# joaospinto/sip_optimal_control

Hardware: AMD Instinct MI355X
Metric: Riccati sweeps/sec (backward+forward) (higher is better)
Workload: dtype f64

## Files before the change

sip_optimal_control_amd/csrc/kkt_chain_kernels.hpp:

```cpp
#pragma once
#include <hip/hip_runtime.h>

#include <cstdint>

#include "kkt_kernels.hpp"

namespace sipamd {
namespace kkt {

struct ChainKkt {
  int n, m, T, cn, gn, cT, gT, ce, ge;
  int node_len, edge_len;
  long model_len;
  int x_dim, y_dim, z_dim;
  int mats_stage, vecs_stage;
  long mats_len, vecs_len;
  int lds_item, lds_tail, lds_rows;
  int split;
  int sym;
};

typedef double d2_t __attribute__((ext_vector_type(2)));

template <int FN, int FM>
// ... 104 lines not shown
    for (int u = 0; u < U; ++u)
      if (tid + u * TPB < n0)
        da[tid + u * TPB] = va[u];
#pragma unroll
    for (int u = 0; u < U; ++u)
      if (tid + u * TPB < n1)
        db[tid + u * TPB] = vb[u];
  } else {
    stage_copy2(d0, s0, l0, tid);
    stage_copy2(d1, s1, l1, tid);
  }
}

typedef double d4_t __attribute__((ext_vector_type(4)));

struct CondenseItem {
  long p;
  int i;
  bool last;
  int c, g, ce, ge, nrows, node_len, edge_len;
  int y_dyn, y_nc, y_ec, z_n, z_e;
  const double *item, *r1, *yinv, *zinv, *b, *b_y, *b_z;
  double *mats, *vecs;
};

template <bool WITH_RHS>
__device__ __forceinline__ CondenseItem condense_item(const ChainKkt &ck, const long p, const int i,
                                                      const double *model_all, const double *r1_all,
                                                      const double *inv_all, double *mats_all, const double *b_all,
                                                      double *vecs_all) {
  CondenseItem it;
  const int n = ck.n, m = ck.m, T = ck.T;
  it.p = p, it.i = i, it.last = i == T;
  it.c = it.last ? ck.cT : ck.cn, it.g = it.last ? ck.gT : ck.gn;
  it.ce = it.last ? 0 : ck.ce, it.ge = it.last ? 0 : ck.ge;
  it.nrows = it.c + it.g + it.ce + it.ge;
  it.node_len = n * n + (it.c + it.g) * n, it.edge_len = it.last ? 0 : ck.edge_len;
  const long kkt = (long)ck.x_dim + ck.y_dim + ck.z_dim;
  it.item = model_all + p * ck.model_len + (long)i * (ck.node_len + ck.edge_len);
  it.r1 = r1_all != nullptr ? r1_all + p * ck.x_dim + i * (n + m) : nullptr;
  it.yinv = inv_all + p * ((long)ck.y_dim + ck.z_dim), it.zinv = it.yinv + ck.y_dim;
  it.y_dyn = i * (n + ck.cn), it.y_nc = it.y_dyn + n, it.y_ec = T * (n + ck.cn) + n + ck.cT + i * ck.ce;
  it.z_n = i * ck.gn, it.z_e = T * ck.gn + ck.gT + i * ck.ge;
  it.b = WITH_RHS ? b_all + p * kkt : nullptr;
  it.b_y = WITH_RHS ? it.b + ck.x_dim : nullptr, it.b_z = WITH_RHS ? it.b_y + ck.y_dim : nullptr;
  it.mats = mats_all + p * ck.mats_len + (long)i * ck.mats_stage;
  it.vecs = WITH_RHS ? vecs_all + p * ck.vecs_len + (long)i * ck.vecs_stage : nullptr;
  return it;
}

__device__ __forceinline__ double condense_rhs_row(const CondenseItem &it, const int k, const double *by,
                                                   const double *bz) {
  if (k < it.c)
    return by[it.y_nc + k];
  if (k < it.c + it.g)
    return bz[it.z_n + (k - it.c)];
  if (k < it.c + it.g + it.ce)
    return by[it.y_ec + (k - it.c - it.g)];
  return bz[it.z_e + (k - it.c - it.g - it.ce)];
}
__device__ __forceinline__ double condense_weight_row(const CondenseItem &it, const int k) {
  if (k < it.c)
    return it.yinv[it.y_nc + k];
  if (k < it.c + it.g)
    return it.zinv[it.z_n + (k - it.c)];
  if (k < it.c + it.g + it.ce)
    return it.yinv[it.y_ec + (k - it.c - it.g)];
  return it.zinv[it.z_e + (k - it.c - it.g - it.ce)];
}

struct CondensePre {
  double w, b, q, dy, d, r1;
};

template <bool WITH_RHS, bool MATS>
__device__ __forceinline__ void condense_prefetch(const ChainKkt &ck, const CondenseItem &it, const int tid,
                                                  CondensePre &pre) {
  const int n = ck.n, m = ck.m;
  pre.w = pre.b = pre.q = pre.dy = pre.d = pre.r1 = 0.0;
  if (tid < it.nrows) {
    pre.w = condense_weight_row(it, tid);
    if (WITH_RHS)
      pre.b = condense_rhs_row(it, tid, it.b_y, it.b_z);
  }
  if (MATS) {
    if (tid < n)
      pre.d = it.yinv[it.y_dyn + tid];
    if (tid < (it.last ? n : n + m))
      pre.r1 = it.r1[tid];
  }
  if (WITH_RHS) {
    if (tid < n) {
      pre.q = it.b[it.i * (n + m) + tid];
      pre.dy = it.b_y[it.y_dyn + tid];
    } else if (!it.last && tid >= 32 && tid - 32 < m) {
      pre.q = it.b[it.i * (n + m) + n + (tid - 32)];
    }
  }
}

template <bool WITH_RHS, bool MATS>
__device__ __forceinline__ void condense_commit(const ChainKkt &ck, const CondenseItem &it, const int tid,
                                                const CondensePre &pre, double *wl, double *wr, double *r1s) {
  if (tid < it.nrows) {
    wl[tid] = pre.w;
    if (WITH_RHS)
      wr[tid] = pre.w * pre.b;
  }
  for (int k = tid + TPB; k < it.nrows; k += TPB) {
    const double wk = condense_weight_row(it, k);
    wl[k] = wk;
    if (WITH_RHS)
      wr[k] = wk * condense_rhs_row(it, k, it.b_y, it.b_z);
  }
  if (MATS && tid < (it.last ? ck.n : ck.n + ck.m))
    r1s[tid] = pre.r1;
}

template <bool WITH_RHS, bool MATS>
__device__ __forceinline__ void condense_compute(const ChainKkt &ck, const CondenseItem &it, const int tid,
                                                 const CondensePre &pre, const double *buf, const double *wl,
                                                 double *wr, const double *r1s, const int ncols_rhs,
                                                 const long b_col_stride, const long vecs_col_stride,
                                                 double *obuf = nullptr) {
  const int n = ck.n, m = ck.m, nn = n * n, nm = n * m;
  const bool last = it.last;
  const int c = it.c, g = it.g, ce = it.ce, ge = it.ge;
  const double *Jc = MATS ? buf + nn : buf, *Jg = Jc + c * n;
  const double *eb = buf + it.node_len;
  const int o_m = nn, o_r = o_m + nm, o_a = o_r + m * m, o_b = o_a + nn, o_j = o_b + nm;
  const double *Jxc = MATS ? eb + o_j : buf + (c + g) * n, *Juc = Jxc + ce * n, *Jxg = Juc + ce * m, *Jug = Jxg + ge * n;
  double *mats = MATS ? obuf : it.mats;

  if (MATS)
  {
    const int li = tid & 15, lg = tid >> 4;
    const int ncols = last ? n : n + m;
    const int nt = (ncols + 15) >> 4;
    const bool sym = ck.sym != 0;
// ... 147 lines not shown
        if (!last) {
          acc = dot_seq<true>(acc, Jxc + ce * tid, wr_e, ce);
          acc = dot_seq<true>(acc, Jxg + ge * tid, wr_e + ce, ge);
        }
        vc[tid] = acc;
        vc[n + tid] = -(col == 0 ? pre.dy : bc_y[it.y_dyn + tid]);
      } else if (!last && tid >= 32 && tid - 32 < m) {
        const int d = tid - 32;
        double acc = -(col == 0 ? pre.q : bc[i * (n + m) + n + d]);
        acc = dot_seq<true>(acc, Juc + ce * d, wr_e, ce);
        acc = dot_seq<true>(acc, Jug + ge * d, wr_e + ce, ge);
        vc[2 * n + d] = acc;
      }
    }
  }
}

#ifndef SIP_KKT_RHS_WAVES
#define SIP_KKT_RHS_WAVES 8
#endif
template <bool WITH_RHS, bool MATS = true, int FN = 0, int FM = 0>
__global__ void __launch_bounds__(TPB) __attribute__((amdgpu_waves_per_eu(FN > 0 && !MATS ? SIP_KKT_RHS_WAVES : 1, 8)))
condense_chain_kernel(const ChainKkt ck_in, const double *__restrict__ model_all, const double *__restrict__ r1_all,
                      const double *__restrict__ inv_all, double *__restrict__ mats_all,
                      const double *__restrict__ b_all, double *__restrict__ vecs_all, long batch,
                      const int32_t *__restrict__ status = nullptr, const int ncols = 1,
                      const long b_col_stride = 0, const long vecs_col_stride = 0) {
  static_assert(MATS || WITH_RHS, "nothing to do");
  const ChainKkt ck = family_dims<FN, FM>(ck_in);
  extern __shared__ double sm[];
  double *buf = sm, *wl = buf + (MATS ? ck.lds_item : ck.lds_tail), *wr = wl + ck.lds_rows,
         *r1s = wr + (long)(MATS || ncols < 1 ? 1 : ncols) * ck.lds_rows;
  double *obuf = r1s + ((ck.n + ck.m + 1) & ~1);
  const long p = blockIdx.x / (ck.T + 1);
  const int i = blockIdx.x - (unsigned)(p * (ck.T + 1));
  if (p >= batch || (!MATS && status != nullptr && status[p] != 0))
    return;
  const int tid = threadIdx.x;
  const CondenseItem it = condense_item<WITH_RHS>(ck, p, i, model_all, r1_all, inv_all, mats_all, b_all, vecs_all);
  CondensePre pre;
  condense_prefetch<WITH_RHS, MATS>(ck, it, tid, pre);
  if (MATS) {
    stage_copy2(buf, it.item, it.node_len + it.edge_len, tid);
  } else {
    const int n = ck.n, m = ck.m, nn = n * n;
    const int o_tail = it.node_len + 2 * nn + 2 * n * m + m * m;
    if (it.last)
      stage_copy2(buf, it.item + nn, (it.c + it.g) * n, tid);
    else
      stage_copy_pair(buf, it.item + nn, (it.c + it.g) * n, buf + (it.c + it.g) * n, it.item + o_tail,
                      (it.ce + it.ge) * (n + m), tid);
  }
  condense_commit<WITH_RHS, MATS>(ck, it, tid, pre, wl, wr, r1s);
  __syncthreads();
  condense_compute<WITH_RHS, MATS>(ck, it, tid, pre, buf, wl, wr, r1s, ncols, b_col_stride, vecs_col_stride, obuf);
}

#ifdef SIP_KKT_STAMPS
__device__ unsigned long long g_kkt_seg[16];
#define KKT_SEG(k)                                                                                   \
  do {                                                                                               \
    const unsigned long long now_ = __builtin_amdgcn_s_memtime();                                    \
    seg[k] += now_ - seg_last;                                                                       \
    seg_last = now_;                                                                                 \
  } while (0)
#else
#define KKT_SEG(k)                                                                                   \
  do {                                                                                               \
  } while (0)
#endif
constexpr int PIPE_U = 8;
#ifndef SIP_KKT_PIPE_WAVES
#define SIP_KKT_PIPE_WAVES 1
#endif
template <bool WITH_RHS, int FN = 0, int FM = 0>
__global__ void __launch_bounds__(TPB) __attribute__((amdgpu_waves_per_eu(FN > 0 ? SIP_KKT_PIPE_WAVES : 1, 8)))
condense_chain_pipe_kernel(const ChainKkt ck_in, const double *__restrict__ model_all,
                           const double *__restrict__ r1_all, const double *__restrict__ inv_all,
                           double *__restrict__ mats_all, const double *__restrict__ b_all,
                           double *__restrict__ vecs_all, const long batch, const int per_block) {
  const ChainKkt ck = family_dims<FN, FM>(ck_in);
  extern __shared__ double sm[];
  double *buf = sm, *wl = buf + ck.lds_item, *wr = wl + ck.lds_rows, *r1s = wr + ck.lds_rows;
  double *obuf = r1s + ((ck.n + ck.m + 1) & ~1);
  const int tid = threadIdx.x;
  const long total = batch * (ck.T + 1);
  const long first = (long)blockIdx.x * per_block;
  const long end = first + per_block < total ? first + per_block : total;
  if (first >= end)
    return;
  long walk_p = first / (ck.T + 1);
  int walk_i = (int)(first - walk_p * (ck.T + 1));
  auto item_here = [&]() {
    return condense_item<WITH_RHS>(ck, walk_p, walk_i, model_all, r1_all, inv_all, mats_all, b_all, vecs_all);
  };
  auto step_walk = [&]() {
    if (++walk_i > ck.T)
      walk_i = 0, ++walk_p;
  };
  const int ab_at = ck.node_len + ck.n * ck.n + ck.n * ck.m + ck.m * ck.m;
  const int ab_first = ck.split ? (ab_at + 1) >> 1 : 0;
  const int ab_end = ck.split ? (ab_at + ck.n * ck.n + ck.n * ck.m) >> 1 : 0;
  auto image_load = [&](const CondenseItem &it, d2_t (&v)[PIPE_U]) {
    typedef d2_t d2u_t __attribute__((aligned(8)));
    const d2u_t *s2 = (const d2u_t *)it.item;
    const int len2 = (it.node_len + it.edge_len + 1) >> 1;
#pragma unroll
    for (int u = 0; u < PIPE_U; ++u) {
      int q = min(tid + u * TPB, len2 - 1);
      if (!it.last && q >= ab_first && q < ab_end)
        q = ab_first - 1;
      v[u] = s2[q];
    }
  };
#ifdef SIP_KKT_STAMPS
  unsigned long long seg[8] = {0, 0, 0, 0, 0, 0, 0, 0}, seg_last = __builtin_amdgcn_s_memtime();
#endif
// ... 23 lines not shown
      condense_prefetch<WITH_RHS, true>(ck, cur, tid, pre);
      image_load(cur, img);
    }
    KKT_SEG(3);
    condense_compute<WITH_RHS, true>(ck, nowit, tid, now, buf, wl, wr, r1s, 1, 0, 0, obuf);
    KKT_SEG(4);
    __syncthreads();
    KKT_SEG(5);
  }
#ifdef SIP_KKT_STAMPS
  if (tid == 0)
    for (int k = 0; k < 8; ++k)
      atomicAdd(&g_kkt_seg[k], seg[k]);
#endif
}

#ifndef SIP_KKT_RECOVER_WAVES
#define SIP_KKT_RECOVER_WAVES 8
#endif
template <bool COLS = false, int FN = 0, int FM = 0>
__global__ void __launch_bounds__(TPB) __attribute__((amdgpu_waves_per_eu(FN > 0 && !COLS ? SIP_KKT_RECOVER_WAVES : 1, 8)))
recover_chain_kernel(const ChainKkt ck_in, const double *__restrict__ model_all, const double *__restrict__ b_all,
                     const double *__restrict__ inv_all, const double *__restrict__ lqr_sol_all,
                     double *__restrict__ sol_all, const int32_t *__restrict__ status, long batch,
                     const int ncols = 1, const long b_col_stride = 0, const long lqr_col_stride = 0,
                     const long sol_col_stride = 0) {
  const ChainKkt ck = family_dims<FN, FM>(ck_in);
  extern __shared__ double sm[];
  const int n = ck.n, m = ck.m, T = ck.T;
  const long p = blockIdx.x / (T + 1);
  const int i = blockIdx.x - (unsigned)(p * (T + 1));
  if (p >= batch || status[p] != 0)
    return;
  const int tid = threadIdx.x;
  const bool last = i == T;
  const int c = last ? ck.cT : ck.cn, g = last ? ck.gT : ck.gn;
  const int ce = last ? 0 : ck.ce, ge = last ? 0 : ck.ge;
  const int nn = n * n, nm = n * m;
  const long kkt = (long)ck.x_dim + ck.y_dim + ck.z_dim;
  const double *item = model_all + p * ck.model_len + (long)i * (ck.node_len + ck.edge_len);
  const double *yinv = inv_all + p * ((long)ck.y_dim + ck.z_dim), *zinv = yinv + ck.y_dim;
  const int y_dyn = i * (n + ck.cn), y_nc = y_dyn + n, y_ec = T * (n + ck.cn) + n + ck.cT + i * ck.ce;
  const int z_n = i * ck.gn, z_e = T * ck.gn + ck.gT + i * ck.ge;
  double *jn = sm, *je = jn + (c + g) * n, *xs = sm + ck.lds_tail, *us = xs + n;
  double pre_x = 0.0, pre_y = 0.0, pre_bn = 0.0, pre_wn = 0.0, pre_be = 0.0, pre_we = 0.0;
  {
    const double *b_y = b_all + p * kkt + ck.x_dim, *b_z = b_y + ck.y_dim;
    const double *ls = lqr_sol_all + p * ck.vecs_len + (long)i * ck.vecs_stage;
    if (tid < n) {
      pre_x = ls[tid];
      pre_y = ls[n + tid];
    } else if (!last && tid >= 32 && tid - 32 < m) {
      pre_x = ls[2 * n + (tid - 32)];
    }
    if (tid < c)
      pre_bn = b_y[y_nc + tid], pre_wn = yinv[y_nc + tid];
    else if (tid < c + g)
// ... 407 lines not shown
```

sip_optimal_control_amd/csrc/kkt_kernels.hpp:

```cpp
#pragma once
#include <hip/hip_runtime.h>

#include <cstdint>

namespace sipamd {
namespace kkt {

constexpr int TPB = 64;

enum Block {
  N_Q = 0, N_JC, N_JG, E_Q, E_M, E_R, E_A, E_B, E_JXC, E_JUC, E_JXG, E_JUG, NUM_BLOCKS
};

struct Meta {
  int E, N, root;
  int x_dim, y_dim, z_dim;
  int theta_dim;
  long model_len, in0_len, in1_len, out_len;
  const int *sd, *cd, *ncd, *ngd, *ecd, *egd, *parent, *child, *in_edge, *child_offsets, *child_edges;
  const int *x_state, *x_control, *y_dyn, *y_node_c, *y_edge_c, *z_node, *z_edge;
  const int *y_is_dyn;
  const long *mo[NUM_BLOCKS];
  int lds_q, lds_item, lds_tail, lds_rows;
  const long *oQ, *od, *oq, *oc, *ox, *oy, *oA, *oB, *oM, *oR, *orr, *ou;
// ... 7 lines not shown
  const long idx = (long)blockIdx.x * blockDim.x + threadIdx.x;
  if (idx >= batch * per)
    return;
  const long p = idx / per;
  const int k = (int)(idx - p * per);
  double reg, out;
  if (k < mt.y_dim) {
    reg = r2[p * mt.y_dim + k];
    out = mt.y_is_dyn[k] ? reg : 1.0 / reg;
  } else {
    const long at = p * mt.z_dim + (k - mt.y_dim);
    reg = w[at] + r3[at];
    out = 1.0 / reg;
  }
  inv[idx] = out;
  if (reg <= 0.0)
    atomicOr(&regstat[p], 1);
}

__global__ void __launch_bounds__(256)
merge_status_kernel(const int *__restrict__ regstat, int32_t *__restrict__ status, long batch, int code) {
  const long p = (long)blockIdx.x * blockDim.x + threadIdx.x;
  if (p < batch && regstat[p] != 0)
    status[p] = code;
}

__device__ __forceinline__ double rank_update(double acc, const double *Ja, int ca, const double *Jb, int cb,
                                              int rows, const double *wgt) {
  for (int k = 0; k < rows; ++k)
    acc += (wgt[k] * Jb[k + (long)rows * cb]) * Ja[k + (long)rows * ca];
  return acc;
}

__global__ void __launch_bounds__(TPB)
condense_kernel(const Meta mt, const double *__restrict__ model_all, const double *__restrict__ r1_all,
                const double *__restrict__ inv_all, double *__restrict__ in0_all, long batch) {
  const int items = mt.N + mt.E;
  const long p = blockIdx.x / items;
  const int item = blockIdx.x - (unsigned)(p * items);
  if (p >= batch)
    return;
  const double *model = model_all + p * mt.model_len;
  const double *r1 = r1_all + p * mt.x_dim;
  const double *yinv = inv_all + p * ((long)mt.y_dim + mt.z_dim), *zinv = yinv + mt.y_dim;
  double *in0 = in0_all + p * mt.in0_len;
  const int tid = threadIdx.x;
// ... 612 lines not shown
```

sip_optimal_control_amd/csrc/sip_kkt_amd.hip:

```cpp
#include "../../include/sip_kkt_amd.h"

#include <hip/hip_runtime.h>

#include <algorithm>
#include <cstdio>
#include <cstdlib>
#include <cstring>
#include <new>
#include <string>
#include <type_traits>
#include <vector>

#include "generic_plan.hpp"
#include "stream_fill.hpp"
#include "kkt_chain_kernels.hpp"
#include "kkt_kernels.hpp"
#include "kkt_theta_kernels.hpp"
#include "kkt_theta_chain_kernels.hpp"

struct sip_kkt_plan {
  int64_t batch = 0;
  int device = 0;
  int E = 0, N = 0, root = 0;
  int input_status = SIP_KKT_INVALID_INPUT;
// ... 128 lines not shown
    break;
  switch (family) {
    SIP_KKT_FAMILY_CASE(4, 1) SIP_KKT_FAMILY_CASE(4, 2) SIP_KKT_FAMILY_CASE(4, 3) SIP_KKT_FAMILY_CASE(4, 4)
    SIP_KKT_FAMILY_CASE(6, 1) SIP_KKT_FAMILY_CASE(6, 2) SIP_KKT_FAMILY_CASE(6, 3) SIP_KKT_FAMILY_CASE(6, 4)
    SIP_KKT_FAMILY_CASE(8, 1) SIP_KKT_FAMILY_CASE(8, 2) SIP_KKT_FAMILY_CASE(8, 3) SIP_KKT_FAMILY_CASE(8, 4)
    SIP_KKT_FAMILY_CASE(12, 1) SIP_KKT_FAMILY_CASE(12, 2) SIP_KKT_FAMILY_CASE(12, 3) SIP_KKT_FAMILY_CASE(12, 4)
  default:
    at(std::integral_constant<int, 0>{}, std::integral_constant<int, 0>{});
  }
#undef SIP_KKT_FAMILY_CASE
}

hipError_t launch_condense(const sip_kkt_plan *p, const Regions &r, const double *model, const double *w,
                           const double *r1, const double *r2, const double *r3, const double *b,
                           hipStream_t s, const bool split = false, const bool sym = false) {
  sipamd::kkt::ChainKkt ck = p->ck;
  if (split) {
    const int n = ck.n, m = ck.m;
    const int qlen = sym ? n * (n + 1) / 2 : n * n, rlen = sym ? m * (m + 1) / 2 : m * m;
    ck.split = 1, ck.sym = sym ? 1 : 0;
    ck.mats_stage = (qlen + n) + (n * m + rlen);
    ck.mats_len = (long)(ck.T + 1) * (qlen + n) + (long)ck.T * (n * m + rlen);
  }
  hipError_t e = sipamd::zero_async(r.reg, (size_t)p->batch * sizeof(int), s);
  if (e != hipSuccess)
    return e;
  const long per = (long)p->y_dim + p->z_dim;
  if (per > 0)
    hipLaunchKernelGGL(sipamd::kkt::weights_kernel, dim3((unsigned)((p->batch * per + 255) / 256)), dim3(256), 0, s,
                       p->meta, w, r2, r3, r.inv, r.reg, (long)p->batch);
  const bool pipe = p->chain_kernels && p->chain_pipe > 0 && ((uintptr_t)model & 7) == 0;
  const bool odd_tail = pipe && ((ck.n * ck.n + (ck.cT + ck.gT) * ck.n) & 1);
  const long pipe_batch = odd_tail ? (long)p->batch - 1 : (long)p->batch;
  const unsigned pipe_grid = pipe ? (unsigned)((pipe_batch * p->N + p->chain_pipe - 1) / p->chain_pipe) : 0u;
  const size_t lds_chain = p->chain_kernels ? sizeof(double) * ((size_t)ck.lds_item + 2 * (size_t)ck.lds_rows +
                                                                 (size_t)even(ck.n + ck.m) + (size_t)ck.mats_stage)
                                            : 0;
  auto one_stage = [&](const long q0, const long nb) {
    const long kkt_len = (long)p->x_dim + p->y_dim + p->z_dim;
    const double *mq = model + q0 * ck.model_len, *r1q = r1 + q0 * p->x_dim, *invq = r.inv + q0 * ((long)p->y_dim + p->z_dim);
    double *in0q = r.in0 + q0 * ck.mats_len;
    if (b != nullptr) {
      const double *bq = b + q0 * kkt_len;
      double *in1q = r.in1 + q0 * ck.vecs_len;
      family_dispatch(p->family, [&](auto fn, auto fm) {
        hipLaunchKernelGGL((sipamd::kkt::condense_chain_kernel<true, true, decltype(fn)::value, decltype(fm)::value>),
                           dim3((unsigned)(nb * p->N)), dim3(sipamd::kkt::TPB), lds_chain, s, ck, mq, r1q, invq, in0q, bq,
                           in1q, nb);
      });
    } else {
      family_dispatch(p->family, [&](auto fn, auto fm) {
        hipLaunchKernelGGL((sipamd::kkt::condense_chain_kernel<false, true, decltype(fn)::value, decltype(fm)::value>),
                           dim3((unsigned)(nb * p->N)), dim3(sipamd::kkt::TPB), lds_chain, s, ck, mq, r1q, invq, in0q,
                           (const double *)nullptr, (double *)nullptr, nb);
      });
    }
  };
  if (pipe) {
    if (pipe_batch > 0 && b != nullptr)
      family_dispatch(p->family, [&](auto fn, auto fm) {
        hipLaunchKernelGGL((sipamd::kkt::condense_chain_pipe_kernel<true, decltype(fn)::value, decltype(fm)::value>),
                           dim3(pipe_grid), dim3(sipamd::kkt::TPB), lds_chain, s, ck, model, r1, r.inv, r.in0, b,
                           r.in1, pipe_batch, p->chain_pipe);
      });
    else if (pipe_batch > 0)
      family_dispatch(p->family, [&](auto fn, auto fm) {
        hipLaunchKernelGGL((sipamd::kkt::condense_chain_pipe_kernel<false, decltype(fn)::value, decltype(fm)::value>),
                           dim3(pipe_grid), dim3(sipamd::kkt::TPB), lds_chain, s, ck, model, r1, r.inv, r.in0,
                           (const double *)nullptr, (double *)nullptr, pipe_batch, p->chain_pipe);
      });
    if (odd_tail)
      one_stage((long)p->batch - 1, 1);
  } else if (p->chain_kernels) {
    one_stage(0, (long)p->batch);
  }
  else if (p->staged && b != nullptr)
    hipLaunchKernelGGL(sipamd::kkt::condense_staged_kernel<true>, dim3(node_grid(p)), dim3(sipamd::kkt::TPB),
                       p->lds_condense, s, p->meta, model, r1, r.inv, r.in0, b, r.in1, (long)p->batch);
  else if (p->staged)
    hipLaunchKernelGGL(sipamd::kkt::condense_staged_kernel<false>, dim3(node_grid(p)), dim3(sipamd::kkt::TPB),
                       p->lds_condense, s, p->meta, model, r1, r.inv, r.in0, (const double *)nullptr,
                       (double *)nullptr, (long)p->batch);
  else
    hipLaunchKernelGGL(sipamd::kkt::condense_kernel, dim3(item_grid(p)), dim3(sipamd::kkt::TPB), 0, s, p->meta,
                       model, r1, r.inv, r.in0, (long)p->batch);
  return hipGetLastError();
}

hipError_t launch_merge(const sip_kkt_plan *p, const Regions &r, int32_t *status, hipStream_t s) {
  hipLaunchKernelGGL(sipamd::kkt::merge_status_kernel, dim3((unsigned)((p->batch + 255) / 256)), dim3(256), 0, s,
                     r.reg, status, (long)p->batch, (int)SIP_KKT_NONPOSITIVE_REGULARIZATION);
  return hipGetLastError();
}

hipError_t launch_rhs_meta(const sip_kkt_plan *p, const Meta &mt, const Regions &r, const double *model,
                           const double *b, const int32_t *status, hipStream_t s) {
  if (p->staged)
    hipLaunchKernelGGL(sipamd::kkt::rhs_staged_kernel, dim3(node_grid(p)), dim3(sipamd::kkt::TPB), p->lds_rhs, s,
                       mt, model, b, r.inv, r.in1, status, (long)p->batch);
  else
    hipLaunchKernelGGL(sipamd::kkt::rhs_kernel, dim3(item_grid(p)), dim3(sipamd::kkt::TPB), 0, s, mt, model, b,
                       r.inv, r.in1, status, (long)p->batch);
  return hipGetLastError();
}

hipError_t launch_rhs(const sip_kkt_plan *p, const Regions &r, const double *model, const double *b,
                      const int32_t *status, hipStream_t s) {
  if (p->chain_kernels)
    family_dispatch(p->family, [&](auto fn, auto fm) {
      hipLaunchKernelGGL((sipamd::kkt::condense_chain_kernel<true, false, decltype(fn)::value, decltype(fm)::value>),
                         dim3(node_grid(p)), dim3(sipamd::kkt::TPB),
                         sizeof(double) * ((size_t)p->ck.lds_tail + 2 * (size_t)p->ck.lds_rows), s, p->ck, model,
                         (const double *)nullptr, r.inv, r.in0, b, r.in1, (long)p->batch, status);
    });
  else if (p->staged)
    hipLaunchKernelGGL(sipamd::kkt::rhs_staged_kernel, dim3(node_grid(p)), dim3(sipamd::kkt::TPB), p->lds_rhs, s,
                       p->meta, model, b, r.inv, r.in1, status, (long)p->batch);
  else
    hipLaunchKernelGGL(sipamd::kkt::rhs_kernel, dim3(item_grid(p)), dim3(sipamd::kkt::TPB), 0, s, p->meta, model,
                       b, r.inv, r.in1, status, (long)p->batch);
  return hipGetLastError();
}

hipError_t launch_recover(const sip_kkt_plan *p, const Regions &r, const double *model, const double *b,
                          double *sol, const int32_t *status, hipStream_t s) {
  if (p->chain_kernels)
    family_dispatch(p->family, [&](auto fn, auto fm) {
      hipLaunchKernelGGL((sipamd::kkt::recover_chain_kernel<false, decltype(fn)::value, decltype(fm)::value>),
                         dim3(node_grid(p)), dim3(sipamd::kkt::TPB), p->lds_chain_recover, s, p->ck, model, b, r.inv, r.out,
                         sol, status, (long)p->batch);
    });
  else if (p->staged)
    hipLaunchKernelGGL(sipamd::kkt::recover_staged_kernel, dim3(node_grid(p)), dim3(sipamd::kkt::TPB),
                       p->lds_recover, s, p->meta, model, b, r.inv, r.out, sol, status, (long)p->batch);
  else
    hipLaunchKernelGGL(sipamd::kkt::recover_kernel, dim3(item_grid(p)), dim3(sipamd::kkt::TPB), 0, s, p->meta,
                       model, b, r.inv, r.out, sol, status, (long)p->batch);
  return hipGetLastError();
}

sipamd::kkt::ApplyIO kkt_vector_io(const sip_kkt_plan *p, int theta_dim, const double *d_x, double *d_y) {
  const long xt = (long)p->x_dim + theta_dim, full = xt + p->y_dim + p->z_dim;
  sipamd::kkt::ApplyIO io;
  io.x_x = d_x, io.x_y = d_x + xt, io.x_z = d_x + xt + p->y_dim;
  io.y_x = d_y, io.y_y = d_y + xt, io.y_z = d_y + xt + p->y_dim;
  io.sx = io.sy = io.sz = full;
  io.parts = sipamd::kkt::AP_ALL;
  return io;
}

int apply_blocks(const sip_kkt_plan *p, const double *d_model, const double *d_theta, const double *d_w,
                 const double *d_r1, const double *d_r2, const double *d_r3, const sipamd::kkt::ApplyIO &io,
                 hipStream_t s, const char *what) {
// ... 165 lines not shown
      return SIP_LQR_OK;
    }
    if (rc == SIP_LQR_OK) {
      g.layout_tree_native();
      p->in0_len = g.in0_len, p->in1_len = 0, p->out_len = g.out_len, p->gain_len = 0;
      lqr_bytes = sip_lqr_tree_work_len(p->tree) * sizeof(double) * (size_t)batch;
      p->name = "tree:general";
    }
  }
  if (rc != SIP_LQR_OK) {
    delete p;
    *out = nullptr;
    return rc;
  }
  size_t cur = 0;
  const size_t B = (size_t)batch * sizeof(double);
  p->at_in0 = cur, cur = align256(cur + B * (size_t)p->in0_len);
  p->at_in1 = p->chain ? cur : p->at_in0;
  if (p->chain)
    cur = align256(cur + B * (size_t)p->in1_len);
  p->at_out = cur, cur = align256(cur + B * (size_t)p->out_len);
  p->at_gain = cur, cur = align256(cur + B * (size_t)p->gain_len);
  p->at_inv = cur, cur = align256(cur + B * (size_t)(p->y_dim + p->z_dim));
  p->at_reg = cur, cur = align256(cur + (size_t)batch * sizeof(int));
  p->at_lqr = cur, cur = align256(cur + lqr_bytes);
  p->work_bytes = cur;
  if (!p->chain)
    p->in1_len = p->in0_len;

  std::vector<int> in_edge(N, -1), child_offsets(N + 1, 0), child_edges(E, 0);
  for (int e = 0; e < E; ++e)
    in_edge[p->children[e]] = e, ++child_offsets[p->parents[e] + 1];
  for (int i = 0; i < N; ++i)
    child_offsets[i + 1] += child_offsets[i];
  {
    std::vector<int> cursor(child_offsets.begin(), child_offsets.end() - 1);
    for (int e = 0; e < E; ++e)
      child_edges[cursor[p->parents[e]]++] = e;
  }

  int lds_q = 0, lds_item = 0, lds_tail = 0, lds_rows = 1;
  for (int i = 0; i < N; ++i) {
    const int n = p->sd[i], cg = p->ncd[i] + p->ngd[i];
    lds_q = std::max(lds_q, n * n), lds_item = std::max(lds_item, n * n + cg * n);
    lds_tail = std::max(lds_tail, cg * n), lds_rows = std::max(lds_rows, std::max(cg, n));
  }
  for (int e = 0; e < E; ++e) {
// ... 248 lines not shown
  if (!d_model || (!d_w && p->z_dim > 0) || !d_r1 || !d_r2 || (!d_r3 && p->z_dim > 0) || !d_work ||
      (kkt > 0 && (!d_b || !d_sol)))
    return SIP_LQR_ERR_INVALID_ARGUMENT;
  sipamd::DeviceGuard on_device(p->device);
  if (on_device.err != hipSuccess)
    return report(on_device.err, "sip_kkt_factor_solve(hipSetDevice)");
  hipStream_t s = (hipStream_t)stream;
  const Regions r = regions(p, d_work);
  const bool fused_rhs = p->staged || p->chain_kernels;
  const long ab_off = (long)p->ck.node_len + p->ck.n * p->ck.n + p->ck.n * p->ck.m + p->ck.m * p->ck.m;
  const long ab_stage = (long)p->ck.node_len + p->ck.edge_len;
  const bool split = p->chain_split && fused_rhs && p->E > 0 && ((uintptr_t)d_model & 7) == 0;
  const bool sym = split && p->chain_sym != nullptr;
  hipError_t e = launch_condense(p, r, d_model, d_w, d_r1, d_r2, d_r3, fused_rhs ? d_b : nullptr, s, split, sym);
  if (e == hipSuccess && !fused_rhs)
    e = launch_rhs(p, r, d_model, d_b, nullptr, s);
  if (e != hipSuccess)
    return report(e, "sip_kkt_factor_solve(condense)");
  const int rc = split ? sip_lqr_factor_solve_split(sym ? p->chain_sym : p->chain, r.in0, d_model + ab_off,
                                                    p->ck.model_len, ab_stage, r.in1, r.out, r.gain, d_status, r.lqr, s)
                       : sip_lqr_factor_solve(p->chain, r.in0, r.in1, r.out, r.gain, d_status, r.lqr, s);
  if (rc != SIP_LQR_OK)
    return rc;
  e = launch_merge(p, r, d_status, s);
  if (e == hipSuccess)
    e = launch_recover(p, r, d_model, d_b, d_sol, d_status, s);
  return report(e, "sip_kkt_factor_solve(recover)");
}

int sip_kkt_add_Kx_to_y(const sip_kkt_plan *p, const double *d_model, const double *d_w, const double *d_r1,
                        const double *d_r2, const double *d_r3, const double *d_x, double *d_y, void *stream) {
  if (p == nullptr || p->input_status != SIP_KKT_SUCCESS)
    return SIP_LQR_ERR_INVALID_ARGUMENT;
  const long kkt = (long)p->x_dim + p->y_dim + p->z_dim;
  if (kkt == 0)
    return SIP_LQR_OK;
  if ((!d_model && p->model_len > 0) || (!d_w && p->z_dim > 0) || (!d_r1 && p->x_dim > 0) ||
      (!d_r2 && p->y_dim > 0) || (!d_r3 && p->z_dim > 0) || !d_x || !d_y)
    return SIP_LQR_ERR_INVALID_ARGUMENT;
  return apply_blocks(p, d_model, nullptr, d_w, d_r1, d_r2, d_r3, kkt_vector_io(p, 0, d_x, d_y), (hipStream_t)stream,
                      "sip_kkt_add_Kx_to_y");
}

#define SIP_KKT_BLOCK_OP(NAME, PART, XS, YS)                                                                 \
  int sip_kkt_add_##NAME##_to_y(const sip_kkt_plan *p, const double *d_model, const double *d_x, double *d_y,  \
                                void *stream) {                                                              \
    return block_op(p, d_model, nullptr, sipamd::kkt::PART, XS, YS, d_x, d_y, (hipStream_t)stream,            \
                    "sip_kkt_add_" #NAME "_to_y");                                                           \
  }                                                                                                          \
// ... 194 lines not shown
    if ((e = hipGetLastError()) != hipSuccess)
      return report(e, "sip_kkt_factor_theta(recover)");
    hipLaunchKernelGGL(sipamd::kkt::theta_schur_reduce_kernel, dim3((unsigned)p->batch), dim3(sipamd::kkt::TPB),
                       sizeof(double) * (size_t)th * th, s, p->N, th, sx, d_r1, (const double *)s_part, t.S, d_status,
                       (long)p->batch, (int)SIP_KKT_THETA_SCHUR_FAILURE);
    return report(hipGetLastError(), "sip_kkt_factor_theta(schur)");
  }
  hipLaunchKernelGGL(sipamd::kkt::theta_jacobian_kernel, dim3(node_grid(p)), dim3(sipamd::kkt::TPB), 0, s, p->meta,
                     p->theta_meta, d_theta, t.J, (long)p->batch);
  if ((e = hipGetLastError()) != hipSuccess)
    return report(e, "sip_kkt_factor_theta(jacobian)");
  if (p->chain_kernels) {
    const Regions r = regions(p, d_work);
    const long colJ = (long)p->batch * skkt, colV = (long)p->batch * p->in1_len;
    const size_t rhs_col_lds = sizeof(double) * (size_t)p->ck.lds_rows;
    const size_t rhs_lds = sizeof(double) * ((size_t)p->ck.lds_tail + 2 * (size_t)p->ck.lds_rows);
    const int rhs_cols = 1 + (int)std::min<size_t>((size_t)(th - 1), (64 * 1024 - rhs_lds) / std::max<size_t>(rhs_col_lds, 1));
    for (int c0 = 0; c0 < th; c0 += rhs_cols) {
      const int nc = std::min(rhs_cols, th - c0);
      family_dispatch(p->family, [&](auto fn, auto fm) {
        hipLaunchKernelGGL((sipamd::kkt::condense_chain_kernel<true, false, decltype(fn)::value, decltype(fm)::value>),
                           dim3(node_grid(p)), dim3(sipamd::kkt::TPB),
                           rhs_lds + rhs_col_lds * (size_t)(nc - 1), s, p->ck, d_model,
                           (const double *)nullptr, r.inv, r.in0, (const double *)t.J + (size_t)c0 * colJ,
                           t.vecs_cols + (size_t)c0 * colV, (long)p->batch, (const int32_t *)d_status, nc, colJ, colV);
      });
    }
    if ((e = hipGetLastError()) != hipSuccess)
      return report(e, "sip_kkt_factor_theta(rhs)");
    rc = sip_lqr_solve_multi(p->chain, r.in0, t.vecs_cols, t.lsol_cols, th, r.gain, r.lqr, t.cws, s);
    if (rc != SIP_LQR_OK)
      return rc;
    const size_t rec_col_lds = sizeof(double) * (size_t)(p->ck.n + p->ck.m);
    const int rec_cols = 1 + (int)std::min<size_t>((size_t)(th - 1), (64 * 1024 - p->lds_chain_recover) / rec_col_lds);
    for (int c0 = 0; c0 < th; c0 += rec_cols) {
      const int nc = std::min(rec_cols, th - c0);
      if (nc > 1)
        family_dispatch(p->family, [&](auto fn, auto fm) {
          hipLaunchKernelGGL((sipamd::kkt::recover_chain_kernel<true, decltype(fn)::value, decltype(fm)::value>),
                             dim3(node_grid(p)), dim3(sipamd::kkt::TPB),
                             p->lds_chain_recover + rec_col_lds * (size_t)(nc - 1), s, p->ck, d_model,
                             (const double *)t.J + (size_t)c0 * colJ, r.inv,
                             (const double *)t.lsol_cols + (size_t)c0 * colV, t.KJ + (size_t)c0 * colJ,
                             (const int32_t *)d_status, (long)p->batch, nc, colJ, colV, colJ);
        });
      else
        family_dispatch(p->family, [&](auto fn, auto fm) {
// ... 108 lines not shown
```

Measured before the change: 12.84 million.

## Fuse regularization weight computation into chain condense and recover kernels

For the chain-kernel path, the separate zero-fill and weights_kernel launches are removed. The condense kernel now computes the inverse regularized weights directly from w, r2 and r3, writes them to the inv buffer, and sets a per-stage nonpositive flag. The merge_status launch is folded into the recover kernel, which ORs the stage flags and writes the status code itself. This cuts two or three launches and one global-memory round trip per solve, in exchange for a larger per-stage flag buffer and extra flag scanning in every recover block.

```diff
diff --git a/sip_optimal_control_amd/csrc/kkt_chain_kernels.hpp b/sip_optimal_control_amd/csrc/kkt_chain_kernels.hpp
--- a/sip_optimal_control_amd/csrc/kkt_chain_kernels.hpp
+++ b/sip_optimal_control_amd/csrc/kkt_chain_kernels.hpp
@@ -150,13 +150,21 @@
   int y_dyn, y_nc, y_ec, z_n, z_e;
   const double *item, *r1, *yinv, *zinv, *b, *b_y, *b_z;
   double *mats, *vecs;
+  const double *r2, *wz, *r3;
+  double *yinv_w, *zinv_w;
+  int *flag;
 };
 
-template <bool WITH_RHS>
+struct CondenseReg {
+  const double *w = nullptr, *r2 = nullptr, *r3 = nullptr;
+  int *flag = nullptr;
+};
+
+template <bool WITH_RHS, bool MATS>
 __device__ __forceinline__ CondenseItem condense_item(const ChainKkt &ck, const long p, const int i,
                                                       const double *model_all, const double *r1_all,
-                                                      const double *inv_all, double *mats_all, const double *b_all,
-                                                      double *vecs_all) {
+                                                      double *inv_all, const CondenseReg &reg, double *mats_all,
+                                                      const double *b_all, double *vecs_all) {
   CondenseItem it;
   const int n = ck.n, m = ck.m, T = ck.T;
   it.p = p, it.i = i, it.last = i == T;
@@ -167,7 +175,11 @@
   const long kkt = (long)ck.x_dim + ck.y_dim + ck.z_dim;
   it.item = model_all + p * ck.model_len + (long)i * (ck.node_len + ck.edge_len);
   it.r1 = r1_all != nullptr ? r1_all + p * ck.x_dim + i * (n + m) : nullptr;
-  it.yinv = inv_all + p * ((long)ck.y_dim + ck.z_dim), it.zinv = it.yinv + ck.y_dim;
+  it.yinv_w = inv_all + p * ((long)ck.y_dim + ck.z_dim), it.zinv_w = it.yinv_w + ck.y_dim;
+  it.yinv = it.yinv_w, it.zinv = it.zinv_w;
+  it.r2 = MATS ? reg.r2 + p * ck.y_dim : nullptr;
+  it.wz = MATS ? reg.w + p * ck.z_dim : nullptr, it.r3 = MATS ? reg.r3 + p * ck.z_dim : nullptr;
+  it.flag = MATS ? reg.flag + p * (T + 1) + i : nullptr;
   it.y_dyn = i * (n + ck.cn), it.y_nc = it.y_dyn + n, it.y_ec = T * (n + ck.cn) + n + ck.cT + i * ck.ce;
   it.z_n = i * ck.gn, it.z_e = T * ck.gn + ck.gT + i * ck.ge;
   it.b = WITH_RHS ? b_all + p * kkt : nullptr;
@@ -197,23 +209,56 @@
   return it.zinv[it.z_e + (k - it.c - it.g - it.ce)];
 }
 
+__device__ __forceinline__ void condense_reg_row(const CondenseItem &it, const int k, double &a, double &b) {
+  b = 0.0;
+  if (k < it.c) {
+    a = it.r2[it.y_nc + k];
+  } else if (k < it.c + it.g) {
+    a = it.wz[it.z_n + (k - it.c)], b = it.r3[it.z_n + (k - it.c)];
+  } else if (k < it.c + it.g + it.ce) {
+    a = it.r2[it.y_ec + (k - it.c - it.g)];
+  } else {
+    a = it.wz[it.z_e + (k - it.c - it.g - it.ce)], b = it.r3[it.z_e + (k - it.c - it.g - it.ce)];
+  }
+}
+__device__ __forceinline__ bool condense_row_ineq(const CondenseItem &it, const int k) {
+  return (k >= it.c && k < it.c + it.g) || k >= it.c + it.g + it.ce;
+}
+__device__ __forceinline__ double *condense_inv_row(const CondenseItem &it, const int k) {
+  if (k < it.c)
+    return it.yinv_w + it.y_nc + k;
+  if (k < it.c + it.g)
+    return it.zinv_w + it.z_n + (k - it.c);
+  if (k < it.c + it.g + it.ce)
+    return it.yinv_w + it.y_ec + (k - it.c - it.g);
+  return it.zinv_w + it.z_e + (k - it.c - it.g - it.ce);
+}
+__device__ __forceinline__ double condense_row_weight(const bool ineq, const double a, const double b, bool &bad) {
+  const double reg = ineq ? a + b : a;
+  bad |= reg <= 0.0;
+  return 1.0 / reg;
+}
+
 struct CondensePre {
-  double w, b, q, dy, d, r1;
+  double w, w3, b, q, dy, d, r1;
 };
 
 template <bool WITH_RHS, bool MATS>
 __device__ __forceinline__ void condense_prefetch(const ChainKkt &ck, const CondenseItem &it, const int tid,
                                                   CondensePre &pre) {
   const int n = ck.n, m = ck.m;
-  pre.w = pre.b = pre.q = pre.dy = pre.d = pre.r1 = 0.0;
+  pre.w = pre.w3 = pre.b = pre.q = pre.dy = pre.d = pre.r1 = 0.0;
   if (tid < it.nrows) {
-    pre.w = condense_weight_row(it, tid);
+    if (MATS)
+      condense_reg_row(it, tid, pre.w, pre.w3);
+    else
+      pre.w = condense_weight_row(it, tid);
     if (WITH_RHS)
       pre.b = condense_rhs_row(it, tid, it.b_y, it.b_z);
   }
   if (MATS) {
     if (tid < n)
-      pre.d = it.yinv[it.y_dyn + tid];
+      pre.d = it.r2[it.y_dyn + tid];
     if (tid < (it.last ? n : n + m))
       pre.r1 = it.r1[tid];
   }
@@ -230,19 +275,42 @@
 template <bool WITH_RHS, bool MATS>
 __device__ __forceinline__ void condense_commit(const ChainKkt &ck, const CondenseItem &it, const int tid,
                                                 const CondensePre &pre, double *wl, double *wr, double *r1s) {
+  bool bad = false;
   if (tid < it.nrows) {
-    wl[tid] = pre.w;
+    double wk = pre.w;
+    if (MATS) {
+      wk = condense_row_weight(condense_row_ineq(it, tid), pre.w, pre.w3, bad);
+      *condense_inv_row(it, tid) = wk;
+    }
+    wl[tid] = wk;
     if (WITH_RHS)
-      wr[tid] = pre.w * pre.b;
+      wr[tid] = wk * pre.b;
   }
   for (int k = tid + TPB; k < it.nrows; k += TPB) {
-    const double wk = condense_weight_row(it, k);
+    double wk;
+    if (MATS) {
+      double a, b;
+      condense_reg_row(it, k, a, b);
+      wk = condense_row_weight(condense_row_ineq(it, k), a, b, bad);
+      *condense_inv_row(it, k) = wk;
+    } else {
+      wk = condense_weight_row(it, k);
+    }
     wl[k] = wk;
     if (WITH_RHS)
       wr[k] = wk * condense_rhs_row(it, k, it.b_y, it.b_z);
   }
-  if (MATS && tid < (it.last ? ck.n : ck.n + ck.m))
-    r1s[tid] = pre.r1;
+  if (MATS) {
+    if (tid < ck.n) {
+      bad |= pre.d <= 0.0;
+      it.yinv_w[it.y_dyn + tid] = pre.d;
+    }
+    if (tid < (it.last ? ck.n : ck.n + ck.m))
+      r1s[tid] = pre.r1;
+    const bool any_bad = __any(bad);
+    if (tid == 0)
+      *it.flag = any_bad ? 1 : 0;
+  }
 }
 
 template <bool WITH_RHS, bool MATS>
@@ -436,7 +504,7 @@
 template <bool WITH_RHS, bool MATS = true, int FN = 0, int FM = 0>
 __global__ void __launch_bounds__(TPB) __attribute__((amdgpu_waves_per_eu(FN > 0 && !MATS ? SIP_KKT_RHS_WAVES : 1, 8)))
 condense_chain_kernel(const ChainKkt ck_in, const double *__restrict__ model_all, const double *__restrict__ r1_all,
-                      const double *__restrict__ inv_all, double *__restrict__ mats_all,
+                      double *__restrict__ inv_all, const CondenseReg reg, double *__restrict__ mats_all,
                       const double *__restrict__ b_all, double *__restrict__ vecs_all, long batch,
                       const int32_t *__restrict__ status = nullptr, const int ncols = 1,
                       const long b_col_stride = 0, const long vecs_col_stride = 0) {
@@ -451,7 +519,7 @@
   if (p >= batch || (!MATS && status != nullptr && status[p] != 0))
     return;
   const int tid = threadIdx.x;
-  const CondenseItem it = condense_item<WITH_RHS>(ck, p, i, model_all, r1_all, inv_all, mats_all, b_all, vecs_all);
+  const CondenseItem it = condense_item<WITH_RHS, MATS>(ck, p, i, model_all, r1_all, inv_all, reg, mats_all, b_all, vecs_all);
   CondensePre pre;
   condense_prefetch<WITH_RHS, MATS>(ck, it, tid, pre);
   if (MATS) {
@@ -490,7 +558,7 @@
 template <bool WITH_RHS, int FN = 0, int FM = 0>
 __global__ void __launch_bounds__(TPB) __attribute__((amdgpu_waves_per_eu(FN > 0 ? SIP_KKT_PIPE_WAVES : 1, 8)))
 condense_chain_pipe_kernel(const ChainKkt ck_in, const double *__restrict__ model_all,
-                           const double *__restrict__ r1_all, const double *__restrict__ inv_all,
+                           const double *__restrict__ r1_all, double *__restrict__ inv_all, const CondenseReg reg,
                            double *__restrict__ mats_all, const double *__restrict__ b_all,
                            double *__restrict__ vecs_all, const long batch, const int per_block) {
   const ChainKkt ck = family_dims<FN, FM>(ck_in);
@@ -506,7 +574,7 @@
   long walk_p = first / (ck.T + 1);
   int walk_i = (int)(first - walk_p * (ck.T + 1));
   auto item_here = [&]() {
-    return condense_item<WITH_RHS>(ck, walk_p, walk_i, model_all, r1_all, inv_all, mats_all, b_all, vecs_all);
+    return condense_item<WITH_RHS, true>(ck, walk_p, walk_i, model_all, r1_all, inv_all, reg, mats_all, b_all, vecs_all);
   };
   auto step_walk = [&]() {
     if (++walk_i > ck.T)
@@ -576,17 +644,33 @@
 __global__ void __launch_bounds__(TPB) __attribute__((amdgpu_waves_per_eu(FN > 0 && !COLS ? SIP_KKT_RECOVER_WAVES : 1, 8)))
 recover_chain_kernel(const ChainKkt ck_in, const double *__restrict__ model_all, const double *__restrict__ b_all,
                      const double *__restrict__ inv_all, const double *__restrict__ lqr_sol_all,
-                     double *__restrict__ sol_all, const int32_t *__restrict__ status, long batch,
+                     double *__restrict__ sol_all, const int32_t *status, long batch,
                      const int ncols = 1, const long b_col_stride = 0, const long lqr_col_stride = 0,
-                     const long sol_col_stride = 0) {
+                     const long sol_col_stride = 0, const int *__restrict__ flag = nullptr,
+                     int32_t *status_out = nullptr, const int flag_code = 0) {
   const ChainKkt ck = family_dims<FN, FM>(ck_in);
   extern __shared__ double sm[];
   const int n = ck.n, m = ck.m, T = ck.T;
   const long p = blockIdx.x / (T + 1);
   const int i = blockIdx.x - (unsigned)(p * (T + 1));
-  if (p >= batch || status[p] != 0)
+  if (p >= batch)
     return;
   const int tid = threadIdx.x;
+  if (flag != nullptr) {
+    int f = 0;
+    for (int k = tid; k <= T; k += TPB)
+      f |= flag[p * (T + 1) + k];
+    const int32_t st = status[p];
+    if (__any(f != 0)) {
+      if (i == 0 && tid == 0)
+        status_out[p] = flag_code;
+      return;
+    }
+    if (st != 0)
+      return;
+  } else if (status[p] != 0) {
+    return;
+  }
   const bool last = i == T;
   const int c = last ? ck.cT : ck.cn, g = last ? ck.gT : ck.gn;
   const int ce = last ? 0 : ck.ce, ge = last ? 0 : ck.ge;
diff --git a/sip_optimal_control_amd/csrc/kkt_kernels.hpp b/sip_optimal_control_amd/csrc/kkt_kernels.hpp
--- a/sip_optimal_control_amd/csrc/kkt_kernels.hpp
+++ b/sip_optimal_control_amd/csrc/kkt_kernels.hpp
@@ -53,6 +53,19 @@
 merge_status_kernel(const int *__restrict__ regstat, int32_t *__restrict__ status, long batch, int code) {
   const long p = (long)blockIdx.x * blockDim.x + threadIdx.x;
   if (p < batch && regstat[p] != 0)
+    status[p] = code;
+}
+
+__global__ void __launch_bounds__(256)
+merge_stage_flags_kernel(const int *__restrict__ flag, const int stages, int32_t *__restrict__ status, long batch,
+                         int code) {
+  const long p = (long)blockIdx.x * blockDim.x + threadIdx.x;
+  if (p >= batch)
+    return;
+  int f = 0;
+  for (int i = 0; i < stages; ++i)
+    f |= flag[p * stages + i];
+  if (f != 0)
     status[p] = code;
 }
 
diff --git a/sip_optimal_control_amd/csrc/sip_kkt_amd.hip b/sip_optimal_control_amd/csrc/sip_kkt_amd.hip
--- a/sip_optimal_control_amd/csrc/sip_kkt_amd.hip
+++ b/sip_optimal_control_amd/csrc/sip_kkt_amd.hip
@@ -174,13 +174,17 @@
     ck.mats_stage = (qlen + n) + (n * m + rlen);
     ck.mats_len = (long)(ck.T + 1) * (qlen + n) + (long)ck.T * (n * m + rlen);
   }
-  hipError_t e = sipamd::zero_async(r.reg, (size_t)p->batch * sizeof(int), s);
-  if (e != hipSuccess)
-    return e;
-  const long per = (long)p->y_dim + p->z_dim;
-  if (per > 0)
-    hipLaunchKernelGGL(sipamd::kkt::weights_kernel, dim3((unsigned)((p->batch * per + 255) / 256)), dim3(256), 0, s,
-                       p->meta, w, r2, r3, r.inv, r.reg, (long)p->batch);
+  if (!p->chain_kernels) {
+    hipError_t e = sipamd::zero_async(r.reg, (size_t)p->batch * sizeof(int), s);
+    if (e != hipSuccess)
+      return e;
+    const long per = (long)p->y_dim + p->z_dim;
+    if (per > 0)
+      hipLaunchKernelGGL(sipamd::kkt::weights_kernel, dim3((unsigned)((p->batch * per + 255) / 256)), dim3(256), 0, s,
+                         p->meta, w, r2, r3, r.inv, r.reg, (long)p->batch);
+  }
+  sipamd::kkt::CondenseReg reg;
+  reg.w = w, reg.r2 = r2, reg.r3 = r3, reg.flag = r.reg;
   const bool pipe = p->chain_kernels && p->chain_pipe > 0 && ((uintptr_t)model & 7) == 0;
   const bool odd_tail = pipe && ((ck.n * ck.n + (ck.cT + ck.gT) * ck.n) & 1);
   const long pipe_batch = odd_tail ? (long)p->batch - 1 : (long)p->batch;
@@ -190,20 +194,23 @@
                                             : 0;
   auto one_stage = [&](const long q0, const long nb) {
     const long kkt_len = (long)p->x_dim + p->y_dim + p->z_dim;
-    const double *mq = model + q0 * ck.model_len, *r1q = r1 + q0 * p->x_dim, *invq = r.inv + q0 * ((long)p->y_dim + p->z_dim);
-    double *in0q = r.in0 + q0 * ck.mats_len;
+    const double *mq = model + q0 * ck.model_len, *r1q = r1 + q0 * p->x_dim;
+    double *invq = r.inv + q0 * ((long)p->y_dim + p->z_dim), *in0q = r.in0 + q0 * ck.mats_len;
+    sipamd::kkt::CondenseReg regq;
+    regq.w = w + q0 * p->z_dim, regq.r2 = r2 + q0 * p->y_dim, regq.r3 = r3 + q0 * p->z_dim;
+    regq.flag = r.reg + q0 * p->N;
     if (b != nullptr) {
       const double *bq = b + q0 * kkt_len;
       double *in1q = r.in1 + q0 * ck.vecs_len;
       family_dispatch(p->family, [&](auto fn, auto fm) {
         hipLaunchKernelGGL((sipamd::kkt::condense_chain_kernel<true, true, decltype(fn)::value, decltype(fm)::value>),
-                           dim3((unsigned)(nb * p->N)), dim3(sipamd::kkt::TPB), lds_chain, s, ck, mq, r1q, invq, in0q, bq,
-                           in1q, nb);
+                           dim3((unsigned)(nb * p->N)), dim3(sipamd::kkt::TPB), lds_chain, s, ck, mq, r1q, invq, regq, in0q,
+                           bq, in1q, nb);
       });
     } else {
       family_dispatch(p->family, [&](auto fn, auto fm) {
         hipLaunchKernelGGL((sipamd::kkt::condense_chain_kernel<false, true, decltype(fn)::value, decltype(fm)::value>),
-                           dim3((unsigned)(nb * p->N)), dim3(sipamd::kkt::TPB), lds_chain, s, ck, mq, r1q, invq, in0q,
+                           dim3((unsigned)(nb * p->N)), dim3(sipamd::kkt::TPB), lds_chain, s, ck, mq, r1q, invq, regq, in0q,
                            (const double *)nullptr, (double *)nullptr, nb);
       });
     }
@@ -212,13 +219,13 @@
     if (pipe_batch > 0 && b != nullptr)
       family_dispatch(p->family, [&](auto fn, auto fm) {
         hipLaunchKernelGGL((sipamd::kkt::condense_chain_pipe_kernel<true, decltype(fn)::value, decltype(fm)::value>),
-                           dim3(pipe_grid), dim3(sipamd::kkt::TPB), lds_chain, s, ck, model, r1, r.inv, r.in0, b,
+                           dim3(pipe_grid), dim3(sipamd::kkt::TPB), lds_chain, s, ck, model, r1, r.inv, reg, r.in0, b,
                            r.in1, pipe_batch, p->chain_pipe);
       });
     else if (pipe_batch > 0)
       family_dispatch(p->family, [&](auto fn, auto fm) {
         hipLaunchKernelGGL((sipamd::kkt::condense_chain_pipe_kernel<false, decltype(fn)::value, decltype(fm)::value>),
-                           dim3(pipe_grid), dim3(sipamd::kkt::TPB), lds_chain, s, ck, model, r1, r.inv, r.in0,
+                           dim3(pipe_grid), dim3(sipamd::kkt::TPB), lds_chain, s, ck, model, r1, r.inv, reg, r.in0,
                            (const double *)nullptr, (double *)nullptr, pipe_batch, p->chain_pipe);
       });
     if (odd_tail)
@@ -240,8 +247,12 @@
 }
 
 hipError_t launch_merge(const sip_kkt_plan *p, const Regions &r, int32_t *status, hipStream_t s) {
-  hipLaunchKernelGGL(sipamd::kkt::merge_status_kernel, dim3((unsigned)((p->batch + 255) / 256)), dim3(256), 0, s,
-                     r.reg, status, (long)p->batch, (int)SIP_KKT_NONPOSITIVE_REGULARIZATION);
+  if (p->chain_kernels)
+    hipLaunchKernelGGL(sipamd::kkt::merge_stage_flags_kernel, dim3((unsigned)((p->batch + 255) / 256)), dim3(256), 0, s,
+                       r.reg, p->N, status, (long)p->batch, (int)SIP_KKT_NONPOSITIVE_REGULARIZATION);
+  else
+    hipLaunchKernelGGL(sipamd::kkt::merge_status_kernel, dim3((unsigned)((p->batch + 255) / 256)), dim3(256), 0, s,
+                       r.reg, status, (long)p->batch, (int)SIP_KKT_NONPOSITIVE_REGULARIZATION);
   return hipGetLastError();
 }
 
@@ -263,7 +274,8 @@
       hipLaunchKernelGGL((sipamd::kkt::condense_chain_kernel<true, false, decltype(fn)::value, decltype(fm)::value>),
                          dim3(node_grid(p)), dim3(sipamd::kkt::TPB),
                          sizeof(double) * ((size_t)p->ck.lds_tail + 2 * (size_t)p->ck.lds_rows), s, p->ck, model,
-                         (const double *)nullptr, r.inv, r.in0, b, r.in1, (long)p->batch, status);
+                         (const double *)nullptr, r.inv, sipamd::kkt::CondenseReg{}, r.in0, b, r.in1, (long)p->batch,
+                         status);
     });
   else if (p->staged)
     hipLaunchKernelGGL(sipamd::kkt::rhs_staged_kernel, dim3(node_grid(p)), dim3(sipamd::kkt::TPB), p->lds_rhs, s,
@@ -275,12 +287,14 @@
 }
 
 hipError_t launch_recover(const sip_kkt_plan *p, const Regions &r, const double *model, const double *b,
-                          double *sol, const int32_t *status, hipStream_t s) {
+                          double *sol, const int32_t *status, hipStream_t s, int32_t *merge_into = nullptr) {
   if (p->chain_kernels)
     family_dispatch(p->family, [&](auto fn, auto fm) {
       hipLaunchKernelGGL((sipamd::kkt::recover_chain_kernel<false, decltype(fn)::value, decltype(fm)::value>),
                          dim3(node_grid(p)), dim3(sipamd::kkt::TPB), p->lds_chain_recover, s, p->ck, model, b, r.inv, r.out,
-                         sol, status, (long)p->batch);
+                         sol, status, (long)p->batch, 1, 0L, 0L, 0L,
+                         (const int *)(merge_into != nullptr ? r.reg : nullptr), merge_into,
+                         (int)SIP_KKT_NONPOSITIVE_REGULARIZATION);
     });
   else if (p->staged)
     hipLaunchKernelGGL(sipamd::kkt::recover_staged_kernel, dim3(node_grid(p)), dim3(sipamd::kkt::TPB),
@@ -492,7 +506,7 @@
   p->at_out = cur, cur = align256(cur + B * (size_t)p->out_len);
   p->at_gain = cur, cur = align256(cur + B * (size_t)p->gain_len);
   p->at_inv = cur, cur = align256(cur + B * (size_t)(p->y_dim + p->z_dim));
-  p->at_reg = cur, cur = align256(cur + (size_t)batch * sizeof(int));
+  p->at_reg = cur, cur = align256(cur + (size_t)batch * (size_t)(p->chain ? N : 1) * sizeof(int));
   p->at_lqr = cur, cur = align256(cur + lqr_bytes);
   p->work_bytes = cur;
   if (!p->chain)
@@ -787,9 +801,13 @@
                        : sip_lqr_factor_solve(p->chain, r.in0, r.in1, r.out, r.gain, d_status, r.lqr, s);
   if (rc != SIP_LQR_OK)
     return rc;
-  e = launch_merge(p, r, d_status, s);
-  if (e == hipSuccess)
-    e = launch_recover(p, r, d_model, d_b, d_sol, d_status, s);
+  if (p->chain_kernels) {
+    e = launch_recover(p, r, d_model, d_b, d_sol, d_status, s, d_status);
+  } else {
+    e = launch_merge(p, r, d_status, s);
+    if (e == hipSuccess)
+      e = launch_recover(p, r, d_model, d_b, d_sol, d_status, s);
+  }
   return report(e, "sip_kkt_factor_solve(recover)");
 }
 
@@ -1030,7 +1048,8 @@
         hipLaunchKernelGGL((sipamd::kkt::condense_chain_kernel<true, false, decltype(fn)::value, decltype(fm)::value>),
                            dim3(node_grid(p)), dim3(sipamd::kkt::TPB),
                            rhs_lds + rhs_col_lds * (size_t)(nc - 1), s, p->ck, d_model,
-                           (const double *)nullptr, r.inv, r.in0, (const double *)t.J + (size_t)c0 * colJ,
+                           (const double *)nullptr, r.inv, sipamd::kkt::CondenseReg{}, r.in0,
+                           (const double *)t.J + (size_t)c0 * colJ,
                            t.vecs_cols + (size_t)c0 * colV, (long)p->batch, (const int32_t *)d_status, nc, colJ, colV);
       });
     }
```

Result: no change. 12.75 million (-0.7%).
